# LeadRDRK/ZPack

Hardware: AMD Instinct MI355X
Metric: decompressed GiB/s over all entries; % HBM roofline (higher is better)
Workload: dtype u8; 1 GPU; c2_lz4_64k; entries_per_gpu=100000, entries_total=100000, archive_image_bytes_this_rank=3543588472, archive_image_bytes_all_ranks=3543588472, method=lz4, level=0, class_mix=70/20/5/5 text/records/random/runs, parallelism=one batch per rank, no data-path collective, rehearsal_one_card=False, frames_by=liblz4/libzstd of the image, reference writer call sequence

## Files before the change

### zpack_amd/__init__.py

```python
import ctypes as C
import os

import numpy as np

HERE = os.path.dirname(os.path.abspath(__file__))
CODEC_SO = os.environ.get("ZPACK_AMD_CODEC_SO") or os.path.join(HERE, "libzpk_codec.so")
ZPACK_SO = os.path.join(HERE, "libzpack_amd.so")

METHOD_NONE, METHOD_ZSTD, METHOD_LZ4 = 0, 1, 2
DF_SKIP_HASH = 1
DF_GENERAL = 2
K_CLASSIFY, K_STORED, K_LZ4, K_ZSTD, K_ZSTD_FSE, K_PACK, K_ENCODE = 0, 1, 2, 3, 4, 5, 7
OPT_ENC_SPLIT_MIN, OPT_DEC_SPLIT_MIN, OPT_ORDER_MIN, OPT_ORDER_FAST_LAST = 6, 7, 8, 9

DECODE_DESC = np.dtype([("src_offset", "<u8"), ("comp_size", "<u8"), ("uncomp_size", "<u8"), ("expect_hash", "<u8"),
                        ("dst_offset", "<u8"), ("dst_capacity", "<u8"), ("method", "<u4"), ("flags", "<u4")])
DECODE_RESULT = np.dtype([("status", "<i4"), ("detail", "<u4"), ("produced", "<u8"), ("hash", "<u8")])
ENCODE_DESC = np.dtype([("src_offset", "<u8"), ("size", "<u8"), ("dst_offset", "<u8"), ("dst_capacity", "<u8"),
                        ("method", "<u4"), ("level", "<i4")])
ENCODE_RESULT = np.dtype([("status", "<i4"), ("detail", "<u4"), ("comp_size", "<u8"), ("hash", "<u8")])
assert DECODE_DESC.itemsize == 56 and DECODE_RESULT.itemsize == 24
assert ENCODE_DESC.itemsize == 40 and ENCODE_RESULT.itemsize == 24

_lib = None
# ... 121 lines not shown
        self._chk(self.L.zpk_codec_set_profiling(self.h, 1 if on else 0), "set_profiling")

    def kernel_ms(self, which):
        ms = C.c_float(0)
        self._chk(self.L.zpk_codec_kernel_ms(self.h, which, C.byref(ms)), "kernel_ms")
        return ms.value

    def decode_stats(self):
        a = (C.c_uint32 * 8)()
        self._chk(self.L.zpk_codec_decode_stats(self.h, a), "decode_stats")
        b = (C.c_uint32 * 16)()
        self.L.zpk_codec_decode_stats2.argtypes = [C.c_void_p, C.POINTER(C.c_uint32)]
        self._chk(self.L.zpk_codec_decode_stats2(self.h, b), "decode_stats2")
        return dict(stored=a[0], zstd=a[1], lz4=a[2], zstd_two_stage=a[3], zstd_fused=a[4], fse_watchdog=a[5], fse_budget=a[6],
                    zstd_arena_refused=bool(a[7] >> 31), retried_lz4=b[0], retried_zstd=b[1],
                    lz4_long_runs=b[3],
                    frame_parallel_entries=b[5], frame_parallel_frames=b[6], zstd_blocks_flags=b[7])

    def debug_fetch(self, what, offset, count, dtype):
        a = np.zeros(count, dtype=dtype)
        self._chk(self.L.zpk_codec_debug_fetch(self.h, what, offset, a.ctypes.data, a.nbytes), "debug_fetch")
        return a

    def debug_read(self, n):
        a = np.zeros((n, 8), dtype=np.uint64)
        self._chk(self.L.zpk_codec_debug_read(self.h, a.ctypes.data, a.nbytes), "debug_read")
        return a

    def timer_start(self, stream=None):
        self._chk(self.L.zpk_codec_timer_start(self.h, C.c_void_p(stream) if stream else None), "timer_start")

# ... 44 lines not shown
```

### zpack_amd/csrc/lz4_wave.h

```cpp
#pragma once
#include "zpk_device.h"
#include "xxh3_device.h"
#include "seq_exec.h"

namespace zpk {

__device__ __noinline__ u32 window_word(const u8* a, const u8* lo, const u8* hi)
{
    if (a >= lo && a + 4 <= hi) return ld32(a);
    u32 v = 0;
    #pragma unroll
    for (int i = 0; i < 4; i++) if (a + i >= lo && a + i < hi) v |= (u32)ld8(a + i) << (8 * i);
    return v;
}

struct ByteWindow {
    u32 w;
    const u8* base;
    const u8* lo;
    const u8* hi;

    __device__ __forceinline__ void load(const u8* p, int lane)
    {
        base = (const u8*)((u64)p & ~(u64)3);
// ... 380 lines not shown
        if (cck) {
            if (iend - ip < 4) { r.rc = D_TRUNCATED; r.produced = (u64)(op - dst); return r; }
            u32 h = 0;
            lane0_guard();
            if (lane == 0) h = xxh32_serial(frame_out, (u64)(op - frame_out), 0);
            if (uni(h) != uld32(ip)) { r.rc = D_MALFORMED; return r; }
            ip += 4;
        }
        if (has_cs && content_size != (u64)(op - frame_out)) { r.rc = D_MALFORMED; return r; }
        if (rs) { rs->nframes++; rs->in_blocks = 0; rs->frame_ip_off = (u64)(ip - src); rs->frame_op_off = (u64)(op - dst); }
    }
    r.produced = (u64)(op - dst);
    return r;
}

}
```

### zpack_amd/csrc/zpk_codec.hip

```cpp
#include <hip/hip_runtime.h>
#include <stdio.h>
#include <stdlib.h>
#include <string.h>
#include <new>
#include <time.h>
#include <pthread.h>
#include <thread>
#include <atomic>
#include <vector>
#include <algorithm>


#include "zpk_device.h"
#include "xxh3_device.h"
#include "xxh3_span.h"
#include "lz4_wave.h"
#include "lx_ring.h"
#ifndef LX_WAVES_PER_SIMD
#define LX_WAVES_PER_SIMD 6
#endif
#include "zstd_wg.h"
#include "zstd_fse4.h"
#include "zstd_ring.h"
#include "lz4_pj.h"
#include "zstd_pj.h"
#include "host_walk.h"

using namespace zpk;

enum { L_NONE = 0, L_ZSTD = 1, L_LZ4 = 2, L_COUNT = 4, N_LISTS = 3, L_LZ4_RUNS = 100  };
enum { C_ZSTD_TWO_STAGE = 9, C_ZSTD_FUSED = 10, C_EXEC_HEAD = 16, C_LEFT_COUNT = 17,
       C_RETRY_LZ4 = 18, C_RETRY_ZSTD = 19,
       C_RETRY_HEAD = 20,
       C_LZ4_LEFT = 21, C_LZ4_LEFT_HEAD = 22,
       C_ENC_CLASS = 28,
       C_ORDER_SPAN = 26,
       C_ORDER = 32,
       N_COUNTERS = 32 + 64 };
enum { N_LISTS_ALLOC = N_LISTS + 5 };


#define ORD_CLASSES 16
__device__ __forceinline__ int order_class(u64 size)
{
    const int lg = 63 - __clzll((long long)(size | 1));
    const int b = 26 - lg;
    return b < 0 ? 0 : (b > ORD_CLASSES - 1 ? ORD_CLASSES - 1 : b);
}
__device__ __forceinline__ int order_fast(u64 size, u64 comp) { return comp * 16 >= size * 15 ? 1 : 0; }
__global__ __launch_bounds__(256) void k_classify(const zpk_decode_desc* __restrict__ desc, u64 n, u64 src_size, u64 dst_size,
                                                  zpk_decode_result* __restrict__ res, u32* __restrict__ lists, u64 list_stride,
                                                  u32* __restrict__ counters)
{
    u64 i = (u64)blockIdx.x * blockDim.x + threadIdx.x;
    const bool live = i < n;
    zpk_decode_desc d; memset(&d, 0, sizeof(d));
    if (live) d = desc[i];
    zpk_decode_result r; r.status = R_OK; r.detail = 0; r.produced = 0; r.hash = 0;
    int list = -1;
    if (!live) list = -1;
    else if (d.comp_size == 0) r.status = R_OK;
    else if (d.dst_capacity < d.uncomp_size) r.status = R_BUFFER_TOO_SMALL;
    else if (d.src_offset + d.comp_size >= src_size || d.src_offset > src_size || d.comp_size > src_size - d.src_offset)
        r.status = R_FILE_OFFSET_INVALID;
    else if (d.dst_offset > dst_size || d.dst_capacity > dst_size - d.dst_offset) { r.status = R_BUFFER_TOO_SMALL; r.detail = 0xBAD0D57u; }
    else if (d.method == ZPK_METHOD_NONE) {
        if (d.uncomp_size > d.comp_size) r.status = R_FILE_SIZE_INVALID;
        else list = L_NONE;
    }
    else if (d.method == ZPK_METHOD_ZSTD) list = L_ZSTD;
    else if (d.method == ZPK_METHOD_LZ4) list = d.comp_size < (d.uncomp_size >> 3) ? L_LZ4_RUNS : L_LZ4;
    else r.status = R_COMP_METHOD_INVALID;
    if (list >= 0) { r.status = R_DECOMPRESS_FAILED; r.detail = 0xFFFFFFFFu; }
    if (live) res[i] = r;
    const int lane = lane_id();
    {
        const bool dec = list == L_ZSTD || list == L_LZ4;
        u32 hi = dec ? (u32)order_class(d.uncomp_size) + 1u : 0u, inv = dec ? (u32)(ORD_CLASSES - order_class(d.uncomp_size)) : 0u;
        #pragma unroll
        for (int m = 1; m < 64; m <<= 1) { const u32 a = (u32)__shfl_xor((int)hi, m, 64), b2 = (u32)__shfl_xor((int)inv, m, 64); hi = a > hi ? a : hi; inv = b2 > inv ? b2 : inv; }
        if (lane == 0 && hi) { atomicMax(&counters[C_ORDER_SPAN], hi - 1u); atomicMax(&counters[C_ORDER_SPAN + 1], inv - 1u); }
    }
    #pragma unroll
    for (int L = 0; L < N_LISTS; L++) {
        const u64 m = __ballot(list == L);
        if (m == 0) continue;
        const int leader = __ffsll((long long)m) - 1;
        u32 base = 0;
        if (lane == leader) base = atomicAdd(&counters[L], (u32)__popcll(m));
        base = (u32)__shfl((int)base, leader, 64);
        if (list == L) lists[(u64)L * list_stride + base + (u32)__popcll(m & ((1ull << lane) - 1))] = (u32)i;
    }
    {
        const u64 m = __ballot(list == L_LZ4_RUNS);
        if (m != 0) {
            const int leader = __ffsll((long long)m) - 1;
            u32 base = 0;
            if (lane == leader) base = atomicAdd(&counters[C_LZ4_LEFT], (u32)__popcll(m));
            base = (u32)__shfl((int)base, leader, 64);
            if (list == L_LZ4_RUNS) lists[(u64)(N_LISTS + 2) * list_stride + base + (u32)__popcll(m & ((1ull << lane) - 1))] = (u32)i;
        }
    }
}

__device__ __forceinline__ bool order_single_class(const u32* counters) { return counters[C_ORDER_SPAN] + counters[C_ORDER_SPAN + 1] == ORD_CLASSES - 1; }
__device__ __forceinline__ void order_wave_rank(int b, int lane, u32& rank, u32& count)
{
    rank = 0; count = 0;
    u64 todo = __ballot(b >= 0);
    while (todo) {
        const int cls = __shfl(b, __ffsll((long long)todo) - 1, 64);
        const u64 m = __ballot(b == cls);
        if (b == cls) { rank = (u32)__popcll(m & ((1ull << lane) - 1)); count = (u32)__popcll(m); }
        todo &= ~m;
    }
}
__global__ __launch_bounds__(256) void k_order_count(const zpk_decode_desc* __restrict__ desc, const u32* __restrict__ lists, u64 list_stride,
                                                     u32* __restrict__ counters, int fast_last)
{
    __shared__ u32 h[ORD_CLASSES];
    const int L = blockIdx.y == 0 ? L_ZSTD : L_LZ4;
    const u32 cnt = counters[L];
    const bool uniform = order_single_class(counters);
    if ((u64)blockIdx.x * 256 >= cnt || (uniform && !fast_last)) return;
    if (threadIdx.x < ORD_CLASSES) h[threadIdx.x] = 0;
    __syncthreads();
    const u64 k = (u64)blockIdx.x * 256 + threadIdx.x;
    const int lane = lane_id();
    int b = -1;
    if (k < cnt) { const zpk_decode_desc& d = desc[lists[(u64)L * list_stride + k]]; b = uniform ? order_fast(d.uncomp_size, d.comp_size) : order_class(d.uncomp_size); }
    u32 rank, count;
    order_wave_rank(b, lane, rank, count);
    if (b >= 0 && rank == 0) atomicAdd(&h[b], count);
    __syncthreads();
    if (threadIdx.x < ORD_CLASSES && h[threadIdx.x]) atomicAdd(&counters[C_ORDER + blockIdx.y * ORD_CLASSES + threadIdx.x], h[threadIdx.x]);
}
__global__ __launch_bounds__(256) void k_order_fill(const zpk_decode_desc* __restrict__ desc, const u32* __restrict__ lists, u64 list_stride,
                                                    u32* __restrict__ ordered , u32* __restrict__ counters, int fast_last)
{
    __shared__ u32 wcount[4][ORD_CLASSES], base[ORD_CLASSES];
    const int L = blockIdx.y == 0 ? L_ZSTD : L_LZ4;
    const u32 cnt = counters[L];
    if ((u64)blockIdx.x * 256 >= cnt) return;
    const u64 k = (u64)blockIdx.x * 256 + threadIdx.x;
    const bool uniform = order_single_class(counters);
    if (uniform && !fast_last) { if (k < cnt) ordered[(u64)blockIdx.y * list_stride + k] = lists[(u64)L * list_stride + k]; return; }
    if (threadIdx.x < 4 * ORD_CLASSES) (&wcount[0][0])[threadIdx.x] = 0;
    __syncthreads();
    const int lane = lane_id(), w = threadIdx.x >> 6;
    u32 e = 0; int b = -1;
    if (k < cnt) { e = lists[(u64)L * list_stride + k]; b = uniform ? order_fast(desc[e].uncomp_size, desc[e].comp_size) : order_class(desc[e].uncomp_size); }
    u32 rank, count;
    order_wave_rank(b, lane, rank, count);
    if (b >= 0 && rank == 0) wcount[w][b] = count;
    __syncthreads();
    if (threadIdx.x < ORD_CLASSES) {
        const int c = threadIdx.x;
        const u32 total = wcount[0][c] + wcount[1][c] + wcount[2][c] + wcount[3][c];
        const u32* const hist = counters + C_ORDER + blockIdx.y * ORD_CLASSES;
        u32 before = 0;
        for (int j = 0; j < c; j++) before += hist[j];
        base[c] = total ? before + atomicAdd(&counters[C_ORDER + 2 * ORD_CLASSES + blockIdx.y * ORD_CLASSES + c], total) : 0;
    }
    __syncthreads();
    if (b >= 0) {
        u32 at = base[b] + rank;
        for (int j = 0; j < w; j++) at += wcount[j][b];
        ordered[(u64)blockIdx.y * list_stride + at] = e;
    }
}

__device__ __forceinline__ bool my_slot(const u32* counters, int list, u32& idx)
{
    idx = uni((u32)(((u64)blockIdx.x * blockDim.x + threadIdx.x) >> 6));
    return idx < uni(counters[list]);
}

__device__ __forceinline__ void finish_entry(const zpk_decode_desc& d, zpk_decode_result* res, u32 e, int status, u32 detail,
                                             u64 produced, const u8* out, int lane)
{
    u64 h = 0;
    lane0_guard();
    if (status == R_OK) {
// ... 46 lines not shown
            const u64 done = nblocks << 10;
            for (u64 i = done + lane; i < len; i += WAVE) st8(out + i, ld8(in + i));
            const u32 nstripes = (u32)(((len - 1) - done) >> 6);
            h = st.finish(in + done, nstripes, in + len, len, lane);
        }
        int status = R_OK;
        if (!(d.flags & ZPK_DF_SKIP_HASH) && h != d.expect_hash) status = R_FILE_HASH_MISMATCH;
        lane0_guard();
        if (lane == 0) {
            zpk_decode_result r; r.status = status; r.detail = 0; r.produced = len; r.hash = h;
            res[e] = r;
        }
    }
}

template <int COOP>
__device__ __forceinline__ void lz4_entry_wave(Lz4WaveShared& shw, const u8* __restrict__ src, const u8* read_lo, const u8* read_hi,
                                               const zpk_decode_desc* __restrict__ desc, u8* dst, zpk_decode_result* __restrict__ res,
                                               u32 e, u32* __restrict__ counters, u64* __restrict__ dbg, u32* __restrict__ retry_list,
                                               u32 wd_scale, int lane)
{
    const zpk_decode_desc d = desc[e];
    const u8* in = uni_ptr(src + d.src_offset);
    u8* out = uni_ptr(dst + d.dst_offset);
    Watchdog wd; wd.arm(uni64(d.comp_size) + uni64(d.dst_capacity), wd_scale);
    SeqStats stt = {};
    const u64 t_all = SEQ_T(); (void)t_all;
    DecodeOut o = lz4f_decode_wave<COOP>(shw, wd, stt, in, uni64(d.comp_size), read_lo, read_hi, out, uni64(d.dst_capacity), lane);
#ifdef ZPK_STATS
    if (dbg && lane == 0) {
        u64* g = dbg + (u64)e * 8;
        g[0] = stt.t_parse; g[1] = stt.t_lit; g[2] = stt.t_dep; g[3] = stt.t_rounds;
        g[4] = ((u64)stt.batches << 32) | stt.rounds; g[5] = ((u64)stt.coops << 32) | stt.asm_batches; g[6] = SEQ_T() - t_all;
        g[7] = ((u64)stt.fix_iters << 32) | stt.chunks;
#ifdef ZPK_STATS_PARSE
        g[0] = stt.t_stage; g[1] = stt.t_walk1; g[2] = stt.t_fix; g[3] = stt.t_emit; g[4] = stt.t_tok;
        g[5] = ((u64)stt.hops_first << 32) | stt.hops_fix; g[6] = stt.slow_hops;
#endif
    }
#else
    (void)dbg; (void)t_all;
#endif
    if (wd.fired && retry_list) {
        lane0_guard();
        if (lane == 0) retry_list[atomicAdd(&counters[C_RETRY_LZ4], 1u)] = e;
        return;
    }
    int status = R_OK;
    if (o.rc == D_MALFORMED) status = R_DECOMPRESS_FAILED;
    else if (o.rc == D_TRUNCATED) status = o.produced < d.dst_capacity ? R_FILE_INCOMPLETE : R_BUFFER_TOO_SMALL;
    else if (o.rc == D_DST_FULL) status = R_BUFFER_TOO_SMALL;
    finish_entry(d, res, e, status, wd.fired ? 0xDEADu : (u32)(-o.rc), o.produced, out, lane);
}

__global__ __launch_bounds__(64, 8) void k_lz4_wave(const u8* __restrict__ src, const u8* read_lo, const u8* read_hi,
                                                  const zpk_decode_desc* __restrict__ desc, u8* dst,
                                                  zpk_decode_result* __restrict__ res, const u32* __restrict__ list,
                                                  u32* __restrict__ counters, u64* __restrict__ dbg, u32* __restrict__ retry_list
#ifdef ZPK_DEVELOPER
                                                  , u32 wd_scale
#endif
                                                  )
{
#ifndef ZPK_DEVELOPER
    const u32 wd_scale = 1u;
#endif
    const int lane = lane_id();
    __shared__ Lz4WaveShared shw;
    u32 idx;
    if (my_slot(counters, L_LZ4, idx))
        lz4_entry_wave<0>(shw, src, read_lo, read_hi, desc, dst, res, uni(list[idx]), counters, dbg, retry_list, wd_scale, lane);
}

__global__ __launch_bounds__(64, 8) void k_lz4_retry(const u8* __restrict__ src, const u8* read_lo, const u8* read_hi,
                                                   const zpk_decode_desc* __restrict__ desc, u8* dst,
                                                   zpk_decode_result* __restrict__ res, const u32* __restrict__ list,
                                                   u32* __restrict__ counters, u64* __restrict__ dbg)
{
    const int lane = lane_id();
    __shared__ Lz4WaveShared shw;
    const u32 n_slots = uni(counters[C_RETRY_LZ4]);
    for (u32 idx = uni((u32)blockIdx.x); idx < n_slots; idx += gridDim.x)
        lz4_entry_wave<2>(shw, src, read_lo, read_hi, desc, dst, res, uni(list[idx]), counters, dbg, nullptr, (u32)ZPK_WATCHDOG_RETRY_SCALE, lane);
}

#define LZ4_LEFT_GRID_MAX 8192u
#ifndef LZ4_LEFT_WAVES
#define LZ4_LEFT_WAVES 8
#endif
__global__ __launch_bounds__(64, LZ4_LEFT_WAVES) void k_lz4_left(const u8* __restrict__ src, const u8* read_lo, const u8* read_hi,
                                                  const zpk_decode_desc* __restrict__ desc, u8* dst,
                                                  zpk_decode_result* __restrict__ res, const u32* __restrict__ list,
                                                  u32* __restrict__ counters, u64* __restrict__ dbg, u32* __restrict__ retry_list, u32 wd_scale)
{
    const int lane = lane_id();
    __shared__ Lz4WaveShared shw;
    const u32 n_slots = uni(counters[C_LZ4_LEFT]);
    if (n_slots == 0) return;
// ... 341 lines not shown
    CodecLock lk(c);
    (void)hipSetDevice(c->device);
    (void)hipStreamSynchronize(c->stream);
    (void)hipGetLastError();
    c->err[0] = 0;
    const u64 keep = 64ull << 20;
    void** bufs[] = { (void**)&c->d_src, (void**)&c->d_dst, (void**)&c->d_zarena, (void**)&c->d_lit };
    u64* caps[] = { &c->src_cap, &c->dst_cap, &c->zarena_cap, &c->lit_cap };
    for (int i = 0; i < 5; i++) if (*bufs[i] && *caps[i] > keep) { (void)hipFree(*bufs[i]); *bufs[i] = nullptr; *caps[i] = 0; }
}
const char* zpk_codec_last_error(const zpk_codec* c) { return c ? c->err : "no codec"; }
int zpk_codec_device(const zpk_codec* c) { return c ? c->device : -1; }

#ifdef ZPK_DEVELOPER
#define ZPK_DEV(x) x
#define ZPK_WD_ARG , wd_scale
#else
#define ZPK_DEV(x)
#define ZPK_WD_ARG
#endif

static int xxh3_spans_launch(zpk_codec* c, const u8* base, const zpk_span* h_spans, u64 nspans, u64 part_blocks, u64* h_hash, hipStream_t st)
{
    if (nspans == 0) return ZPK_OK;
    if (nspans > 0x7FFFFFFFull) return ZPK_E_INVALID;
    const u64 span_bytes = (nspans * sizeof(zpk_span) + 255) & ~255ull, part_bytes = part_blocks * 64;
    int rc;
    if ((rc = grow(c, (void**)&c->d_xpart, &c->xpart_cap, span_bytes + part_bytes + nspans * 8 + 64))) return rc;
    zpk_span* d_spans = (zpk_span*)c->d_xpart;
    u64* d_part = (u64*)(c->d_xpart + span_bytes);
    u64* d_hash = (u64*)(c->d_xpart + span_bytes + part_bytes);
// ... 7 lines not shown
}
static inline u64 xxh3_span_blocks(u64 len) { return (((len - 1) >> 10) + XS_GROUP - 1) / XS_GROUP * XS_GROUP; }

static int decode_launch(zpk_codec* c, const u8* src, u64 src_size, const u8* read_lo, const u8* read_hi,
                         const zpk_decode_desc* desc, u64 n, u8* dst, u64 dst_size, zpk_decode_result* res, hipStream_t st)
{
    if (n == 0) return ZPK_OK;
    if (n > 0x7FFFFFF0ull) return ZPK_E_INVALID;
    c->totals_valid = 0;
    int rc;
    if ((rc = grow(c, (void**)&c->d_lists, &c->list_cap, N_LISTS_ALLOC * n * sizeof(u32)))) return rc;
    const u64 stride = c->list_cap / (N_LISTS_ALLOC * sizeof(u32));
    u32* const retry_lz4 = c->d_lists + (u64)N_LISTS * stride;
    u32* const retry_zstd = c->d_lists + (u64)(N_LISTS + 1) * stride;
    u32* const left_lz4 = c->d_lists + (u64)(N_LISTS + 2) * stride;
    u32 wd_scale = 1; (void)wd_scale;
    ZPK_DEV(static const int wd_env = getenv("ZPK_WD_SCALE") ? atoi(getenv("ZPK_WD_SCALE")) : 1; wd_scale = (u32)wd_env;)
    int skip = 0; (void)skip;
#ifdef ZPK_DEVELOPER
    static const int want_dbg = getenv("ZPK_DEBUG_TIMING") ? atoi(getenv("ZPK_DEBUG_TIMING")) : 0;
    if (want_dbg) { if ((rc = grow(c, (void**)&c->d_dbg, &c->dbg_cap, n * 128))) return rc; }
    static const int trace = getenv("ZPK_TRACE") ? atoi(getenv("ZPK_TRACE")) : 0;
    static const int skip_env = getenv("ZPK_SKIP") ? atoi(getenv("ZPK_SKIP")) : 0;
    skip = skip_env;
#define ZPK_TRACE_STEP(name) do { if (trace == 1) { hipError_t te_ = hipStreamSynchronize(st); \
        fprintf(stderr, "[zpk] %s done: %s\n", name, hipGetErrorString(te_)); fflush(stderr); } } while (0)
#else
#define ZPK_TRACE_STEP(name) do { } while (0)
#endif
    const u32 zstd_grid = (u32)(n < ZSTD_GRID_MAX ? n : ZSTD_GRID_MAX);
    const u32 exec_grid = (u32)(n < ZSTD_EXEC_GRID_MAX ? n : ZSTD_EXEC_GRID_MAX);
    const bool maybe_zstd = c->zstd_hint != 0;
    if (maybe_zstd && (rc = grow(c, (void**)&c->d_lit, &c->lit_cap, (u64)(exec_grid > zstd_grid ? exec_grid : zstd_grid) * ZSTD_LIT_SCRATCH))) return rc;
    HIPCHK(c, hipMemsetAsync(c->d_counters, 0, N_COUNTERS * sizeof(u32), st));
    ZPK_TRACE_STEP("memset");
#define ZPK_KEV(k, j) do { if (c->profiling) (void)hipEventRecord(c->kev[k][j], st); } while (0)
    ZPK_KEV(ZPK_K_CLASSIFY, 0);
    hipLaunchKernelGGL(k_classify, dim3((u32)((n + 255) / 256)), dim3(256), 0, st, desc, n, src_size, dst_size, res,
                       c->d_lists, stride, c->d_counters);
    const u32* zstd_list = c->d_lists + L_ZSTD * stride;
    const u32* lz4_list = c->d_lists + L_LZ4 * stride;
    if (n >= c->order_min) {
        u32* const ordered = c->d_lists + (u64)(N_LISTS + 3) * stride;
        const dim3 og((u32)((n + 255) / 256), 2);
        hipLaunchKernelGGL(k_order_count, og, dim3(256), 0, st, desc, (const u32*)c->d_lists, stride, c->d_counters, c->order_fast_last);
        hipLaunchKernelGGL(k_order_fill, og, dim3(256), 0, st, desc, (const u32*)c->d_lists, stride, ordered, c->d_counters, c->order_fast_last);
        zstd_list = ordered; lz4_list = ordered + stride;
    }
    ZPK_KEV(ZPK_K_CLASSIFY, 1);
    ZPK_TRACE_STEP("k_classify");
    const u32 wgrid = (u32)((n + 3) / 4);
    ZPK_KEV(ZPK_K_STORED, 0);
    if (!(skip & 1)) hipLaunchKernelGGL(k_stored, dim3(wgrid), dim3(256), 0, st, src, desc, dst, res, c->d_lists + L_NONE * stride, c->d_counters);
    ZPK_KEV(ZPK_K_STORED, 1);
    ZPK_TRACE_STEP("k_stored");
    const bool maybe_lz4 = c->lz4_hint != 0;
    hipStream_t sl = st;
#ifndef ZPK_NO_SIDE_STREAM
    if (!c->h_seen && hipHostMalloc((void**)&c->h_seen, 64, hipHostMallocDefault) == hipSuccess) { c->h_seen[L_NONE] = 0; c->h_seen[L_ZSTD] = 1; c->h_seen[L_LZ4] = 1; c->h_seen[8] = 1; }
    const bool both_seen = c->zstd_hint >= 0  || (c->h_seen && c->h_seen[L_ZSTD] != 0 && c->h_seen[L_LZ4] != 0);
    if (maybe_lz4 && maybe_zstd && both_seen && !(skip & 6)) {
        int lo_prio = 0, hi_prio = 0;
        if (!c->s_side) { (void)hipDeviceGetStreamPriorityRange(&lo_prio, &hi_prio);
                          if (hipStreamCreateWithPriority(&c->s_side, hipStreamNonBlocking, lo_prio) != hipSuccess) c->s_side = nullptr; }
        if (!c->ev_fork && hipEventCreateWithFlags(&c->ev_fork, hipEventDisableTiming) != hipSuccess) c->ev_fork = nullptr;
        if (!c->ev_join && hipEventCreateWithFlags(&c->ev_join, hipEventDisableTiming) != hipSuccess) c->ev_join = nullptr;
        if (c->s_side && c->ev_fork && c->ev_join && hipEventRecord(c->ev_fork, st) == hipSuccess &&
            hipStreamWaitEvent(c->s_side, c->ev_fork, 0) == hipSuccess) sl = c->s_side;
    }
#endif
    auto launch_lz4 = [&]() {
        if (c->profiling) (void)hipEventRecord(c->kev[ZPK_K_LZ4][0], sl);
        if (!(skip & 2) && maybe_lz4) {
            hipStream_t sx = sl;
            if (n >= 4096 && c->h_seen && c->h_seen[8] != 0) {
            if (!c->s_left && hipStreamCreateWithFlags(&c->s_left, hipStreamNonBlocking) != hipSuccess) c->s_left = nullptr;
            if (!c->ev_lfork && hipEventCreateWithFlags(&c->ev_lfork, hipEventDisableTiming) != hipSuccess) c->ev_lfork = nullptr;
            if (!c->ev_ljoin && hipEventCreateWithFlags(&c->ev_ljoin, hipEventDisableTiming) != hipSuccess) c->ev_ljoin = nullptr;
            if (c->s_left && c->ev_lfork && c->ev_ljoin && hipEventRecord(c->ev_lfork, sl) == hipSuccess &&
                hipStreamWaitEvent(c->s_left, c->ev_lfork, 0) == hipSuccess) sx = c->s_left;
            }
            hipLaunchKernelGGL(k_lz4_left, dim3((u32)(n < LZ4_LEFT_GRID_MAX ? n : LZ4_LEFT_GRID_MAX)), dim3(64), 0, sx, src, read_lo, read_hi, desc, dst, res,
                               (const u32*)left_lz4, c->d_counters, c->d_dbg, retry_lz4, wd_scale);
            hipLaunchKernelGGL(k_lz4_wave, dim3((u32)n), dim3(64), 0, sl, src, read_lo, read_hi, desc, dst, res,
                               lz4_list, c->d_counters, c->d_dbg, retry_lz4 ZPK_WD_ARG);
            if (sx != sl && (hipEventRecord(c->ev_ljoin, sx) != hipSuccess || hipStreamWaitEvent(sl, c->ev_ljoin, 0) != hipSuccess))
                (void)hipStreamSynchronize(sx);
            hipLaunchKernelGGL(k_lz4_retry, dim3((u32)(n < 256 ? n : 256)), dim3(64), 0, sl, src, read_lo, read_hi, desc, dst, res,
                               (const u32*)retry_lz4, c->d_counters, c->d_dbg);
        }
        if (c->profiling) (void)hipEventRecord(c->kev[ZPK_K_LZ4][1], sl);
    };
    if (sl == st) launch_lz4();
    ZPK_TRACE_STEP("k_lz4_wave");
    bool two_stage = maybe_zstd && dst_size >= 64;
    ZPK_DEV(static const int fused_only = getenv("ZPK_ZSTD_FUSED") ? atoi(getenv("ZPK_ZSTD_FUSED")) : 0; if (fused_only) two_stage = false;)
    c->fell_back_fused = 0;
    if (two_stage && (grow(c, (void**)&c->d_zarena, &c->zarena_cap, dst_size + 64) != ZPK_OK ||
                      grow(c, (void**)&c->d_zstate, &c->zstate_cap, 2 * n * sizeof(u32)) != ZPK_OK)) {
        two_stage = false; c->fell_back_fused = 1;
        snprintf(c->err, sizeof(c->err), "note: no memory for the %llu-byte Zstandard sequence arena; this batch ran the fused decoder",
                 (unsigned long long)dst_size + 64);
    }
    u32* const leftover = two_stage ? c->d_zstate + n : nullptr;
// ... 15 lines not shown
                       two_stage ? (const u32*)leftover : zstd_list, c->d_counters, c->d_lit, c->d_dbg,
                       two_stage ? (int)C_LEFT_COUNT : (int)L_ZSTD, (int)(L_COUNT + L_ZSTD), retry_zstd, (int)C_RETRY_ZSTD, wd_scale);
    ZPK_KEV(ZPK_K_ZSTD, 1);
    ZPK_TRACE_STEP("k_zstd");
    if (!(skip & 4) && maybe_zstd)
        hipLaunchKernelGGL(k_zstd, dim3(zstd_grid < 128 ? zstd_grid : 128), dim3(ZSTD_WG_THREADS), 0, st, src, desc, dst, res,
                           (const u32*)retry_zstd, c->d_counters, c->d_lit, c->d_dbg, (int)C_RETRY_ZSTD, (int)C_RETRY_HEAD,
                           (u32*)nullptr, 0, (u32)ZPK_WATCHDOG_RETRY_SCALE);
    if (sl != st) {
        launch_lz4();
        if (hipEventRecord(c->ev_join, sl) != hipSuccess || hipStreamWaitEvent(st, c->ev_join, 0) != hipSuccess) {
            (void)hipStreamSynchronize(sl);
        }
    }
    ZPK_TRACE_STEP("retry");
    if (c->h_seen && c->zstd_hint < 0) (void)hipMemcpyAsync((void*)c->h_seen, c->d_counters, N_LISTS * sizeof(u32), hipMemcpyDeviceToHost, st);
    if (c->h_seen) (void)hipMemcpyAsync((void*)(c->h_seen + 8), c->d_counters + C_LZ4_LEFT, sizeof(u32), hipMemcpyDeviceToHost, st);
    HIPCHK(c, hipGetLastError());
    return ZPK_OK;
}

int zpk_codec_decode_batch_device(zpk_codec* c, const uint8_t* src, uint64_t src_size, const zpk_decode_desc* desc, uint64_t n,
                                  uint8_t* dst, uint64_t dst_size, zpk_decode_result* results, void* stream)
{
    if (!c || (n && (!desc || !results))) return ZPK_E_INVALID;
    CodecLock lk(c);
    HIPCHK(c, hipSetDevice(c->device));
    hipStream_t st = stream ? (hipStream_t)stream : c->stream;
    c->zstd_hint = -1; c->lz4_hint = -1;
    return decode_launch(c, src, src_size, src, src + src_size, desc, n, dst, dst_size, results, st);
}
// ... 869 lines not shown
{
    if (!c || !c->d_dbg || bytes > c->dbg_cap) return ZPK_E_INVALID;
    HIPCHK(c, hipDeviceSynchronize());
    HIPCHK(c, hipMemcpy(host, c->d_dbg, bytes, hipMemcpyDeviceToHost));
    return ZPK_OK;
}

int zpk_codec_decode_stats(zpk_codec* c, uint32_t out[8])
{
    if (!c || !out) return ZPK_E_INVALID;
    HIPCHK(c, hipSetDevice(c->device));
    HIPCHK(c, hipDeviceSynchronize());
    u32 h[N_COUNTERS];
    HIPCHK(c, hipMemcpy(h, c->d_counters, sizeof(h), hipMemcpyDeviceToHost));
    if (c->totals_valid) memcpy(h, c->host_totals, sizeof(h));
    out[0] = h[L_NONE]; out[1] = h[L_ZSTD]; out[2] = h[L_LZ4] + h[C_LZ4_LEFT] ; out[3] = h[C_ZSTD_TWO_STAGE]; out[4] = h[C_ZSTD_FUSED];
    out[5] = h[ZF_WATCHDOG_WORD]; out[6] = h[ZF_WATCHDOG_WORD + 1]; out[7] = h[13];
    if (c->fell_back_fused) out[7] |= 0x80000000u;
    ZPK_DEV(if (getenv("ZPK_TRACE")) fprintf(stderr, "[zpk] fse marked %u, pass-0 failures %u, last failure status/rc %08x\n", h[13], h[14], h[15]);)
    return ZPK_OK;
}

int zpk_codec_decode_stats2(zpk_codec* c, uint32_t out[16])
{
    if (!c || !out) return ZPK_E_INVALID;
    CodecLock lk(c);
    HIPCHK(c, hipSetDevice(c->device));
    HIPCHK(c, hipDeviceSynchronize());
    u32 h[N_COUNTERS];
    HIPCHK(c, hipMemcpy(h, c->d_counters, sizeof(h), hipMemcpyDeviceToHost));
    if (c->totals_valid) memcpy(h, c->host_totals, sizeof(h));
    memset(out, 0, 16 * sizeof(uint32_t));
    out[0] = h[C_RETRY_LZ4]; out[1] = h[C_RETRY_ZSTD];
    out[2] = 0; out[3] = h[C_LZ4_LEFT]; out[4] = 0;
    out[5] = c->big_last[0]; out[6] = c->big_last[1];
    out[7] = c->zpj_last_err;
    return ZPK_OK;
}

int zpk_codec_debug_fetch(zpk_codec* c, int what, uint64_t offset, void* host, uint64_t bytes)
{
    if (!c || !host) return ZPK_E_INVALID;
    const u8* base = what == 0 ? (const u8*)c->d_zarena : (const u8*)c->d_zstate;
    const u64 cap = what == 0 ? c->zarena_cap : c->zstate_cap;
    if (!base || offset > cap || bytes > cap - offset) return ZPK_E_INVALID;
    HIPCHK(c, hipSetDevice(c->device));
    HIPCHK(c, hipDeviceSynchronize());
    HIPCHK(c, hipMemcpy(host, base + offset, bytes, hipMemcpyDeviceToHost));
    return ZPK_OK;
}

// ... 52 lines not shown
```

Measured before the change: 624.6 GiB/s.

## Split LZ4 decode into lean plain-frame path and general fallback kernel

Classification now inspects each LZ4 frame header and sends common plain frames (no checksums, no dict, default flags) to a slimmed k_lz4_wave that uses a specialized lz4f_plain_wave decoder. Other frames go to a new k_lz4_general persistent kernel. Entries the lean path rejects are handed to the retry kernel, which now drains three queues. The goal is less per-entry branching and register pressure on the common path, at the cost of an extra kernel launch, more list slots and counters, and a reading of source headers during classification.

```diff
diff --git a/zpack_amd/__init__.py b/zpack_amd/__init__.py
--- a/zpack_amd/__init__.py
+++ b/zpack_amd/__init__.py
@@ -159,7 +159,7 @@
         self._chk(self.L.zpk_codec_decode_stats2(self.h, b), "decode_stats2")
         return dict(stored=a[0], zstd=a[1], lz4=a[2], zstd_two_stage=a[3], zstd_fused=a[4], fse_watchdog=a[5], fse_budget=a[6],
                     zstd_arena_refused=bool(a[7] >> 31), retried_lz4=b[0], retried_zstd=b[1],
-                    lz4_long_runs=b[3],
+                    lz4_long_runs=b[3], lz4_handed_over=b[8], lz4_general=b[9],
                     frame_parallel_entries=b[5], frame_parallel_frames=b[6], zstd_blocks_flags=b[7])
 
     def debug_fetch(self, what, offset, count, dtype):
diff --git a/zpack_amd/csrc/lz4_wave.h b/zpack_amd/csrc/lz4_wave.h
--- a/zpack_amd/csrc/lz4_wave.h
+++ b/zpack_amd/csrc/lz4_wave.h
@@ -418,4 +418,51 @@
     return r;
 }
 
-}
+template <int COOP = 0>
+__device__ inline bool lz4f_plain_wave(Lz4WaveShared& sh, Watchdog& wd, SeqStats& stt, const u8* src, u64 src_size, const u8* src_hi,
+                                       u8* dst, u64 dst_cap, u64 want, int lane)
+{
+    if (src_size < 11) return false;
+    if (uld32(src) != 0x184D2204u) return false;
+    const u32 flg = uld8(src + 4), bd = uld8(src + 5);
+    if ((flg & 0xD7u) != 0x40u || (bd & 0x8Fu) || ((bd >> 4) & 7u) < 4u) return false;
+    const u32 hdr = (flg & 8u) ? 15u : 7u;
+    if (src_size < hdr + 4u) return false;
+    if ((flg & 8u) && uni64(ld64(src + 6)) != want) return false;
+    {
+        u32 h = 0;
+        lane0_guard();
+        if (lane == 0) h = (xxh32_serial(src + 4, hdr - 5, 0) >> 8) & 0xFF;
+        if (uni(h) != uld8(src + hdr - 1)) return false;
+    }
+    const u64 bmax = (u64)1 << (8 + 2 * ((bd >> 4) & 7u));
+    const bool indep = (flg >> 5) & 1;
+    const u8* ip = src + hdr;
+    const u8* const iend = src + src_size;
+    u8* op = dst;
+    u8* const oend = dst + dst_cap;
+    for (;;) {
+        if (wd.expired() || iend - ip < 4) return false;
+        const u32 bh = uld32(ip);
+        ip += 4;
+        if (bh == 0) break;
+        const u32 bsz = bh & 0x7FFFFFFFu;
+        if (bsz > bmax || (u64)(iend - ip) < bsz) return false;
+        if (bh >> 31) {
+            if (bsz > (u64)(oend - op)) return false;
+            for (u32 i = (u32)lane * 16; i < bsz; i += WAVE * 16) gcopy_upto16(op + i, ip + i, bsz - i < 16 ? bsz - i : 16);
+            op += bsz;
+        } else {
+            u8* hist_lo = indep ? op : dst;
+            if ((u64)(op - hist_lo) > 65536) hist_lo = op - 65536;
+            u8* bend = oend;
+            if ((u64)(oend - op) > bmax) bend = op + bmax;
+            if (lz4_block_wave<COOP>(sh, wd, stt, ip, bsz, src_hi, hist_lo, op, bend, lane) != D_OK) return false;
+        }
+        wave_mem_fence();
+        ip += bsz;
+    }
+    return ip == iend && (u64)(op - dst) == want;
+}
+
+}
diff --git a/zpack_amd/csrc/zpk_codec.hip b/zpack_amd/csrc/zpk_codec.hip
--- a/zpack_amd/csrc/zpk_codec.hip
+++ b/zpack_amd/csrc/zpk_codec.hip
@@ -28,16 +28,24 @@
 
 using namespace zpk;
 
-enum { L_NONE = 0, L_ZSTD = 1, L_LZ4 = 2, L_COUNT = 4, N_LISTS = 3, L_LZ4_RUNS = 100  };
+enum { L_NONE = 0, L_ZSTD = 1, L_LZ4 = 2, L_COUNT = 4, N_LISTS = 3, L_LZ4_RUNS = 100 ,
+       L_LZ4_GEN = 101  };
 enum { C_ZSTD_TWO_STAGE = 9, C_ZSTD_FUSED = 10, C_EXEC_HEAD = 16, C_LEFT_COUNT = 17,
        C_RETRY_LZ4 = 18, C_RETRY_ZSTD = 19,
        C_RETRY_HEAD = 20,
        C_LZ4_LEFT = 21, C_LZ4_LEFT_HEAD = 22,
+       C_LZ4_GEN = 3, C_LZ4_GEN_HEAD = 7,
+       C_LZ4_HANDED_HEAD = 23, C_LZ4_HANDED = 24,
+       C_LZ4_RETRY_HEAD = 25,
        C_ENC_CLASS = 28,
        C_ORDER_SPAN = 26,
        C_ORDER = 32,
-       N_COUNTERS = 32 + 64 };
-enum { N_LISTS_ALLOC = N_LISTS + 5 };
+       N_COUNTERS = 32 + 96 };
+enum { S_LZ4_HANDED = N_LISTS + 5, S_LZ4_GEN = N_LISTS + 6, S_LZ4_GEN_ORDERED = N_LISTS + 7, N_LISTS_ALLOC = N_LISTS + 8 };
+#define N_ORDERED 3
+__device__ __forceinline__ int order_list_slot(int y) { return y == 0 ? (int)L_ZSTD : y == 1 ? (int)L_LZ4 : (int)S_LZ4_GEN; }
+__device__ __forceinline__ int order_count_word(int y) { return y == 0 ? (int)L_ZSTD : y == 1 ? (int)L_LZ4 : (int)C_LZ4_GEN; }
+__device__ __forceinline__ int order_out_slot(int y) { return y == 2 ? (int)S_LZ4_GEN_ORDERED : (int)N_LISTS + 3 + y; }
 
 
 #define ORD_CLASSES 16
@@ -48,7 +56,13 @@
     return b < 0 ? 0 : (b > ORD_CLASSES - 1 ? ORD_CLASSES - 1 : b);
 }
 __device__ __forceinline__ int order_fast(u64 size, u64 comp) { return comp * 16 >= size * 15 ? 1 : 0; }
-__global__ __launch_bounds__(256) void k_classify(const zpk_decode_desc* __restrict__ desc, u64 n, u64 src_size, u64 dst_size,
+__device__ __forceinline__ bool lz4_header_is_plain(const u8* __restrict__ p, u64 comp_size)
+{
+    if (comp_size < 11) return false;
+    const u32 magic = (u32)p[0] | ((u32)p[1] << 8) | ((u32)p[2] << 16) | ((u32)p[3] << 24), flg = p[4], bd = p[5];
+    return magic == 0x184D2204u && (flg & 0xD7u) == 0x40u && (bd & 0x8Fu) == 0 && ((bd >> 4) & 7u) >= 4u;
+}
+__global__ __launch_bounds__(256) void k_classify(const u8* __restrict__ src, const zpk_decode_desc* __restrict__ desc, u64 n, u64 src_size, u64 dst_size,
                                                   zpk_decode_result* __restrict__ res, u32* __restrict__ lists, u64 list_stride,
                                                   u32* __restrict__ counters)
 {
@@ -69,13 +83,14 @@
         else list = L_NONE;
     }
     else if (d.method == ZPK_METHOD_ZSTD) list = L_ZSTD;
-    else if (d.method == ZPK_METHOD_LZ4) list = d.comp_size < (d.uncomp_size >> 3) ? L_LZ4_RUNS : L_LZ4;
+    else if (d.method == ZPK_METHOD_LZ4)
+        list = d.comp_size < (d.uncomp_size >> 3) ? L_LZ4_RUNS : lz4_header_is_plain(src + d.src_offset, d.comp_size) ? L_LZ4 : L_LZ4_GEN;
     else r.status = R_COMP_METHOD_INVALID;
     if (list >= 0) { r.status = R_DECOMPRESS_FAILED; r.detail = 0xFFFFFFFFu; }
     if (live) res[i] = r;
     const int lane = lane_id();
     {
-        const bool dec = list == L_ZSTD || list == L_LZ4;
+        const bool dec = list == L_ZSTD || list == L_LZ4 || list == L_LZ4_GEN;
         u32 hi = dec ? (u32)order_class(d.uncomp_size) + 1u : 0u, inv = dec ? (u32)(ORD_CLASSES - order_class(d.uncomp_size)) : 0u;
         #pragma unroll
         for (int m = 1; m < 64; m <<= 1) { const u32 a = (u32)__shfl_xor((int)hi, m, 64), b2 = (u32)__shfl_xor((int)inv, m, 64); hi = a > hi ? a : hi; inv = b2 > inv ? b2 : inv; }
@@ -101,6 +116,16 @@
             if (list == L_LZ4_RUNS) lists[(u64)(N_LISTS + 2) * list_stride + base + (u32)__popcll(m & ((1ull << lane) - 1))] = (u32)i;
         }
     }
+    {
+        const u64 m = __ballot(list == L_LZ4_GEN);
+        if (m != 0) {
+            const int leader = __ffsll((long long)m) - 1;
+            u32 base = 0;
+            if (lane == leader) base = atomicAdd(&counters[C_LZ4_GEN], (u32)__popcll(m));
+            base = (u32)__shfl((int)base, leader, 64);
+            if (list == L_LZ4_GEN) lists[(u64)S_LZ4_GEN * list_stride + base + (u32)__popcll(m & ((1ull << lane) - 1))] = (u32)i;
+        }
+    }
 }
 
 __device__ __forceinline__ bool order_single_class(const u32* counters) { return counters[C_ORDER_SPAN] + counters[C_ORDER_SPAN + 1] == ORD_CLASSES - 1; }
@@ -119,8 +144,8 @@
                                                      u32* __restrict__ counters, int fast_last)
 {
     __shared__ u32 h[ORD_CLASSES];
-    const int L = blockIdx.y == 0 ? L_ZSTD : L_LZ4;
-    const u32 cnt = counters[L];
+    const int L = order_list_slot(blockIdx.y);
+    const u32 cnt = counters[order_count_word(blockIdx.y)];
     const bool uniform = order_single_class(counters);
     if ((u64)blockIdx.x * 256 >= cnt || (uniform && !fast_last)) return;
     if (threadIdx.x < ORD_CLASSES) h[threadIdx.x] = 0;
@@ -136,15 +161,16 @@
     if (threadIdx.x < ORD_CLASSES && h[threadIdx.x]) atomicAdd(&counters[C_ORDER + blockIdx.y * ORD_CLASSES + threadIdx.x], h[threadIdx.x]);
 }
 __global__ __launch_bounds__(256) void k_order_fill(const zpk_decode_desc* __restrict__ desc, const u32* __restrict__ lists, u64 list_stride,
-                                                    u32* __restrict__ ordered , u32* __restrict__ counters, int fast_last)
+                                                    u32* __restrict__ all_lists , u32* __restrict__ counters, int fast_last)
 {
     __shared__ u32 wcount[4][ORD_CLASSES], base[ORD_CLASSES];
-    const int L = blockIdx.y == 0 ? L_ZSTD : L_LZ4;
-    const u32 cnt = counters[L];
+    const int L = order_list_slot(blockIdx.y);
+    const u32 cnt = counters[order_count_word(blockIdx.y)];
+    u32* const ordered = all_lists + (u64)order_out_slot(blockIdx.y) * list_stride;
     if ((u64)blockIdx.x * 256 >= cnt) return;
     const u64 k = (u64)blockIdx.x * 256 + threadIdx.x;
     const bool uniform = order_single_class(counters);
-    if (uniform && !fast_last) { if (k < cnt) ordered[(u64)blockIdx.y * list_stride + k] = lists[(u64)L * list_stride + k]; return; }
+    if (uniform && !fast_last) { if (k < cnt) ordered[k] = lists[(u64)L * list_stride + k]; return; }
     if (threadIdx.x < 4 * ORD_CLASSES) (&wcount[0][0])[threadIdx.x] = 0;
     __syncthreads();
     const int lane = lane_id(), w = threadIdx.x >> 6;
@@ -160,13 +186,13 @@
         const u32* const hist = counters + C_ORDER + blockIdx.y * ORD_CLASSES;
         u32 before = 0;
         for (int j = 0; j < c; j++) before += hist[j];
-        base[c] = total ? before + atomicAdd(&counters[C_ORDER + 2 * ORD_CLASSES + blockIdx.y * ORD_CLASSES + c], total) : 0;
+        base[c] = total ? before + atomicAdd(&counters[C_ORDER + N_ORDERED * ORD_CLASSES + blockIdx.y * ORD_CLASSES + c], total) : 0;
     }
     __syncthreads();
     if (b >= 0) {
         u32 at = base[b] + rank;
         for (int j = 0; j < w; j++) at += wcount[j][b];
-        ordered[(u64)blockIdx.y * list_stride + at] = e;
+        ordered[at] = e;
     }
 }
 
@@ -243,19 +269,8 @@
     }
 }
 
-template <int COOP>
-__device__ __forceinline__ void lz4_entry_wave(Lz4WaveShared& shw, const u8* __restrict__ src, const u8* read_lo, const u8* read_hi,
-                                               const zpk_decode_desc* __restrict__ desc, u8* dst, zpk_decode_result* __restrict__ res,
-                                               u32 e, u32* __restrict__ counters, u64* __restrict__ dbg, u32* __restrict__ retry_list,
-                                               u32 wd_scale, int lane)
-{
-    const zpk_decode_desc d = desc[e];
-    const u8* in = uni_ptr(src + d.src_offset);
-    u8* out = uni_ptr(dst + d.dst_offset);
-    Watchdog wd; wd.arm(uni64(d.comp_size) + uni64(d.dst_capacity), wd_scale);
-    SeqStats stt = {};
-    const u64 t_all = SEQ_T(); (void)t_all;
-    DecodeOut o = lz4f_decode_wave<COOP>(shw, wd, stt, in, uni64(d.comp_size), read_lo, read_hi, out, uni64(d.dst_capacity), lane);
+__device__ __forceinline__ void lz4_stats_out(u64* __restrict__ dbg, u32 e, const SeqStats& stt, u64 t_all, int lane)
+{
 #ifdef ZPK_STATS
     if (dbg && lane == 0) {
         u64* g = dbg + (u64)e * 8;
@@ -268,8 +283,24 @@
 #endif
     }
 #else
-    (void)dbg; (void)t_all;
-#endif
+    (void)dbg; (void)e; (void)stt; (void)t_all; (void)lane;
+#endif
+}
+
+template <int COOP>
+__device__ __forceinline__ void lz4_entry_wave(Lz4WaveShared& shw, const u8* __restrict__ src, const u8* read_lo, const u8* read_hi,
+                                               const zpk_decode_desc* __restrict__ desc, u8* dst, zpk_decode_result* __restrict__ res,
+                                               u32 e, u32* __restrict__ counters, u64* __restrict__ dbg, u32* __restrict__ retry_list,
+                                               u32 wd_scale, int lane)
+{
+    const zpk_decode_desc d = desc[e];
+    const u8* in = uni_ptr(src + d.src_offset);
+    u8* out = uni_ptr(dst + d.dst_offset);
+    Watchdog wd; wd.arm(uni64(d.comp_size) + uni64(d.dst_capacity), wd_scale);
+    SeqStats stt = {};
+    const u64 t_all = SEQ_T(); (void)t_all;
+    DecodeOut o = lz4f_decode_wave<COOP>(shw, wd, stt, in, uni64(d.comp_size), read_lo, read_hi, out, uni64(d.dst_capacity), lane);
+    lz4_stats_out(dbg, e, stt, t_all, lane);
     if (wd.fired && retry_list) {
         lane0_guard();
         if (lane == 0) retry_list[atomicAdd(&counters[C_RETRY_LZ4], 1u)] = e;
@@ -282,35 +313,102 @@
     finish_entry(d, res, e, status, wd.fired ? 0xDEADu : (u32)(-o.rc), o.produced, out, lane);
 }
 
-__global__ __launch_bounds__(64, 8) void k_lz4_wave(const u8* __restrict__ src, const u8* read_lo, const u8* read_hi,
+__device__ __forceinline__ void lz4_entry_plain(Lz4WaveShared& shw, const u8* __restrict__ src, const u8* read_hi,
+                                                const zpk_decode_desc* __restrict__ desc, u8* dst, zpk_decode_result* __restrict__ res,
+                                                u32 e, u32* __restrict__ counters, u64* __restrict__ dbg, u32* __restrict__ retry_list,
+                                                u32* __restrict__ handed_list, u32 wd_scale, int lane)
+{
+    const zpk_decode_desc& d = desc[e];
+    const u8* in = uni_ptr(src + d.src_offset);
+    u8* out = uni_ptr(dst + d.dst_offset);
+    Watchdog wd; wd.arm(uni64(d.comp_size) + uni64(d.dst_capacity), wd_scale);
+    SeqStats stt = {};
+    const u64 t_all = SEQ_T(); (void)t_all;
+    const bool done = lz4f_plain_wave<0>(shw, wd, stt, in, uni64(d.comp_size), read_hi, out, uni64(d.dst_capacity), uni64(d.uncomp_size), lane);
+    lz4_stats_out(dbg, e, stt, t_all, lane);
+    if (!done) {
+        lane0_guard();
+        if (lane == 0) {
+            if (wd.fired) retry_list[atomicAdd(&counters[C_RETRY_LZ4], 1u)] = e;
+            else handed_list[atomicAdd(&counters[C_LZ4_HANDED], 1u)] = e;
+        }
+        return;
+    }
+    finish_entry(d, res, e, R_OK, 0u, uni64(d.uncomp_size), out, lane);
+}
+
+__global__ __launch_bounds__(64, 8) void k_lz4_wave(const u8* __restrict__ src, const u8* read_hi,
                                                   const zpk_decode_desc* __restrict__ desc, u8* dst,
                                                   zpk_decode_result* __restrict__ res, const u32* __restrict__ list,
-                                                  u32* __restrict__ counters, u64* __restrict__ dbg, u32* __restrict__ retry_list
+                                                  u32* __restrict__ counters, u32* __restrict__ retry_list, u32* __restrict__ handed_list
 #ifdef ZPK_DEVELOPER
-                                                  , u32 wd_scale
+                                                  , u64* __restrict__ dbg, u32 wd_scale
 #endif
                                                   )
 {
 #ifndef ZPK_DEVELOPER
     const u32 wd_scale = 1u;
+    u64* const dbg = nullptr;
 #endif
     const int lane = lane_id();
     __shared__ Lz4WaveShared shw;
     u32 idx;
     if (my_slot(counters, L_LZ4, idx))
+        lz4_entry_plain(shw, src, read_hi, desc, dst, res, uni(list[idx]), counters, dbg, retry_list, handed_list, wd_scale, lane);
+}
+
+#ifdef ZPK_DEVELOPER
+__global__ __launch_bounds__(256) void k_lz4_hand_all(const u32* __restrict__ list, u32* __restrict__ counters, u32* __restrict__ handed_list)
+{
+    const u64 i = (u64)blockIdx.x * blockDim.x + threadIdx.x;
+    if (i < counters[L_LZ4]) handed_list[atomicAdd(&counters[C_LZ4_HANDED], 1u)] = list[i];
+}
+#endif
+
+#define LZ4_GENERAL_GRID_MAX 8192u
+__global__ __launch_bounds__(64, 8) void k_lz4_general(const u8* __restrict__ src, const u8* read_lo, const u8* read_hi,
+                                                     const zpk_decode_desc* __restrict__ desc, u8* dst,
+                                                     zpk_decode_result* __restrict__ res, const u32* __restrict__ list,
+                                                     u32* __restrict__ counters, u64* __restrict__ dbg, u32* __restrict__ retry_list, u32 wd_scale)
+{
+    const int lane = lane_id();
+    __shared__ Lz4WaveShared shw;
+    const u32 n_slots = uni(counters[C_LZ4_GEN]);
+    if (n_slots == 0) return;
+    for (;;) {
+        lane0_guard();
+        u32 v = 0;
+        if (lane == 0) v = atomicAdd(&counters[C_LZ4_GEN_HEAD], 1u);
+        const u32 idx = uni(v);
+        lane0_guard();
+        if (idx >= n_slots) break;
         lz4_entry_wave<0>(shw, src, read_lo, read_hi, desc, dst, res, uni(list[idx]), counters, dbg, retry_list, wd_scale, lane);
+    }
 }
 
 __global__ __launch_bounds__(64, 8) void k_lz4_retry(const u8* __restrict__ src, const u8* read_lo, const u8* read_hi,
                                                    const zpk_decode_desc* __restrict__ desc, u8* dst,
-                                                   zpk_decode_result* __restrict__ res, const u32* __restrict__ list,
-                                                   u32* __restrict__ counters, u64* __restrict__ dbg)
+                                                   zpk_decode_result* __restrict__ res, const u32* __restrict__ lists, u64 list_stride,
+                                                   u32* __restrict__ counters, u64* __restrict__ dbg, int gen_slot)
 {
     const int lane = lane_id();
     __shared__ Lz4WaveShared shw;
-    const u32 n_slots = uni(counters[C_RETRY_LZ4]);
-    for (u32 idx = uni((u32)blockIdx.x); idx < n_slots; idx += gridDim.x)
-        lz4_entry_wave<2>(shw, src, read_lo, read_hi, desc, dst, res, uni(list[idx]), counters, dbg, nullptr, (u32)ZPK_WATCHDOG_RETRY_SCALE, lane);
+    for (int k = 0; k < 3; k++) {
+        const int count_word = k == 0 ? (int)C_LZ4_GEN : k == 1 ? (int)C_LZ4_HANDED : (int)C_RETRY_LZ4;
+        const int head_word = k == 0 ? (int)C_LZ4_GEN_HEAD : k == 1 ? (int)C_LZ4_HANDED_HEAD : (int)C_LZ4_RETRY_HEAD;
+        const u32* const list = lists + (u64)(k == 0 ? gen_slot : k == 1 ? (int)S_LZ4_HANDED : (int)N_LISTS) * list_stride;
+        const u32 n_slots = uni(counters[count_word]);
+        if (n_slots == 0 || uni(counters[head_word]) >= n_slots) continue;
+        for (;;) {
+            lane0_guard();
+            u32 v = 0;
+            if (lane == 0) v = atomicAdd(&counters[head_word], 1u);
+            const u32 idx = uni(v);
+            lane0_guard();
+            if (idx >= n_slots) break;
+            lz4_entry_wave<2>(shw, src, read_lo, read_hi, desc, dst, res, uni(list[idx]), counters, dbg, nullptr, (u32)ZPK_WATCHDOG_RETRY_SCALE, lane);
+        }
+    }
 }
 
 #define LZ4_LEFT_GRID_MAX 8192u
@@ -682,7 +780,7 @@
 
 #ifdef ZPK_DEVELOPER
 #define ZPK_DEV(x) x
-#define ZPK_WD_ARG , wd_scale
+#define ZPK_WD_ARG , c->d_dbg, wd_scale
 #else
 #define ZPK_DEV(x)
 #define ZPK_WD_ARG
@@ -720,6 +818,7 @@
     u32* const retry_lz4 = c->d_lists + (u64)N_LISTS * stride;
     u32* const retry_zstd = c->d_lists + (u64)(N_LISTS + 1) * stride;
     u32* const left_lz4 = c->d_lists + (u64)(N_LISTS + 2) * stride;
+    u32* const handed_lz4 = c->d_lists + (u64)S_LZ4_HANDED * stride;
     u32 wd_scale = 1; (void)wd_scale;
     ZPK_DEV(static const int wd_env = getenv("ZPK_WD_SCALE") ? atoi(getenv("ZPK_WD_SCALE")) : 1; wd_scale = (u32)wd_env;)
     int skip = 0; (void)skip;
@@ -742,17 +841,19 @@
     ZPK_TRACE_STEP("memset");
 #define ZPK_KEV(k, j) do { if (c->profiling) (void)hipEventRecord(c->kev[k][j], st); } while (0)
     ZPK_KEV(ZPK_K_CLASSIFY, 0);
-    hipLaunchKernelGGL(k_classify, dim3((u32)((n + 255) / 256)), dim3(256), 0, st, desc, n, src_size, dst_size, res,
+    hipLaunchKernelGGL(k_classify, dim3((u32)((n + 255) / 256)), dim3(256), 0, st, src, desc, n, src_size, dst_size, res,
                        c->d_lists, stride, c->d_counters);
     const u32* zstd_list = c->d_lists + L_ZSTD * stride;
     const u32* lz4_list = c->d_lists + L_LZ4 * stride;
+    int gen_slot = S_LZ4_GEN;
     if (n >= c->order_min) {
-        u32* const ordered = c->d_lists + (u64)(N_LISTS + 3) * stride;
-        const dim3 og((u32)((n + 255) / 256), 2);
+        const dim3 og((u32)((n + 255) / 256), N_ORDERED);
         hipLaunchKernelGGL(k_order_count, og, dim3(256), 0, st, desc, (const u32*)c->d_lists, stride, c->d_counters, c->order_fast_last);
-        hipLaunchKernelGGL(k_order_fill, og, dim3(256), 0, st, desc, (const u32*)c->d_lists, stride, ordered, c->d_counters, c->order_fast_last);
-        zstd_list = ordered; lz4_list = ordered + stride;
-    }
+        hipLaunchKernelGGL(k_order_fill, og, dim3(256), 0, st, desc, (const u32*)c->d_lists, stride, c->d_lists, c->d_counters, c->order_fast_last);
+        zstd_list = c->d_lists + (u64)(N_LISTS + 3) * stride; lz4_list = c->d_lists + (u64)(N_LISTS + 4) * stride;
+        gen_slot = S_LZ4_GEN_ORDERED;
+    }
+    const u32* const gen_list = c->d_lists + (u64)gen_slot * stride;
     ZPK_KEV(ZPK_K_CLASSIFY, 1);
     ZPK_TRACE_STEP("k_classify");
     const u32 wgrid = (u32)((n + 3) / 4);
@@ -763,8 +864,8 @@
     const bool maybe_lz4 = c->lz4_hint != 0;
     hipStream_t sl = st;
 #ifndef ZPK_NO_SIDE_STREAM
-    if (!c->h_seen && hipHostMalloc((void**)&c->h_seen, 64, hipHostMallocDefault) == hipSuccess) { c->h_seen[L_NONE] = 0; c->h_seen[L_ZSTD] = 1; c->h_seen[L_LZ4] = 1; c->h_seen[8] = 1; }
-    const bool both_seen = c->zstd_hint >= 0  || (c->h_seen && c->h_seen[L_ZSTD] != 0 && c->h_seen[L_LZ4] != 0);
+    if (!c->h_seen && hipHostMalloc((void**)&c->h_seen, 64, hipHostMallocDefault) == hipSuccess) { c->h_seen[L_NONE] = 0; c->h_seen[L_ZSTD] = 1; c->h_seen[L_LZ4] = 1; c->h_seen[8] = 1; c->h_seen[C_LZ4_GEN] = 1; }
+    const bool both_seen = c->zstd_hint >= 0  || (c->h_seen && c->h_seen[L_ZSTD] != 0 && (c->h_seen[L_LZ4] != 0 || c->h_seen[C_LZ4_GEN] != 0));
     if (maybe_lz4 && maybe_zstd && both_seen && !(skip & 6)) {
         int lo_prio = 0, hi_prio = 0;
         if (!c->s_side) { (void)hipDeviceGetStreamPriorityRange(&lo_prio, &hi_prio);
@@ -788,12 +889,21 @@
             }
             hipLaunchKernelGGL(k_lz4_left, dim3((u32)(n < LZ4_LEFT_GRID_MAX ? n : LZ4_LEFT_GRID_MAX)), dim3(64), 0, sx, src, read_lo, read_hi, desc, dst, res,
                                (const u32*)left_lz4, c->d_counters, c->d_dbg, retry_lz4, wd_scale);
-            hipLaunchKernelGGL(k_lz4_wave, dim3((u32)n), dim3(64), 0, sl, src, read_lo, read_hi, desc, dst, res,
-                               lz4_list, c->d_counters, c->d_dbg, retry_lz4 ZPK_WD_ARG);
+            bool lean = true;
+#ifdef ZPK_DEVELOPER
+            static const int all_general = getenv("ZPK_LZ4_GENERAL") ? atoi(getenv("ZPK_LZ4_GENERAL")) : 0;
+            lean = !all_general;
+            if (!lean) hipLaunchKernelGGL(k_lz4_hand_all, dim3((u32)((n + 255) / 256)), dim3(256), 0, sl, lz4_list, c->d_counters, handed_lz4);
+#endif
+            if (lean) hipLaunchKernelGGL(k_lz4_wave, dim3((u32)n), dim3(64), 0, sl, src, read_hi, desc, dst, res,
+                                         lz4_list, c->d_counters, retry_lz4, handed_lz4 ZPK_WD_ARG);
+            if (!c->h_seen || c->h_seen[C_LZ4_GEN] != 0)
+                hipLaunchKernelGGL(k_lz4_general, dim3((u32)(n < LZ4_GENERAL_GRID_MAX ? n : LZ4_GENERAL_GRID_MAX)), dim3(64), 0, sl, src, read_lo, read_hi,
+                                   desc, dst, res, gen_list, c->d_counters, c->d_dbg, retry_lz4, wd_scale);
             if (sx != sl && (hipEventRecord(c->ev_ljoin, sx) != hipSuccess || hipStreamWaitEvent(sl, c->ev_ljoin, 0) != hipSuccess))
                 (void)hipStreamSynchronize(sx);
             hipLaunchKernelGGL(k_lz4_retry, dim3((u32)(n < 256 ? n : 256)), dim3(64), 0, sl, src, read_lo, read_hi, desc, dst, res,
-                               (const u32*)retry_lz4, c->d_counters, c->d_dbg);
+                               (const u32*)c->d_lists, stride, c->d_counters, c->d_dbg, gen_slot);
         }
         if (c->profiling) (void)hipEventRecord(c->kev[ZPK_K_LZ4][1], sl);
     };
@@ -839,7 +949,7 @@
         }
     }
     ZPK_TRACE_STEP("retry");
-    if (c->h_seen && c->zstd_hint < 0) (void)hipMemcpyAsync((void*)c->h_seen, c->d_counters, N_LISTS * sizeof(u32), hipMemcpyDeviceToHost, st);
+    if (c->h_seen && c->zstd_hint < 0) (void)hipMemcpyAsync((void*)c->h_seen, c->d_counters, (N_LISTS + 1) * sizeof(u32), hipMemcpyDeviceToHost, st);
     if (c->h_seen) (void)hipMemcpyAsync((void*)(c->h_seen + 8), c->d_counters + C_LZ4_LEFT, sizeof(u32), hipMemcpyDeviceToHost, st);
     HIPCHK(c, hipGetLastError());
     return ZPK_OK;
@@ -1739,7 +1849,7 @@
     u32 h[N_COUNTERS];
     HIPCHK(c, hipMemcpy(h, c->d_counters, sizeof(h), hipMemcpyDeviceToHost));
     if (c->totals_valid) memcpy(h, c->host_totals, sizeof(h));
-    out[0] = h[L_NONE]; out[1] = h[L_ZSTD]; out[2] = h[L_LZ4] + h[C_LZ4_LEFT] ; out[3] = h[C_ZSTD_TWO_STAGE]; out[4] = h[C_ZSTD_FUSED];
+    out[0] = h[L_NONE]; out[1] = h[L_ZSTD]; out[2] = h[L_LZ4] + h[C_LZ4_LEFT] + h[C_LZ4_GEN] ; out[3] = h[C_ZSTD_TWO_STAGE]; out[4] = h[C_ZSTD_FUSED];
     out[5] = h[ZF_WATCHDOG_WORD]; out[6] = h[ZF_WATCHDOG_WORD + 1]; out[7] = h[13];
     if (c->fell_back_fused) out[7] |= 0x80000000u;
     ZPK_DEV(if (getenv("ZPK_TRACE")) fprintf(stderr, "[zpk] fse marked %u, pass-0 failures %u, last failure status/rc %08x\n", h[13], h[14], h[15]);)
@@ -1760,6 +1870,8 @@
     out[2] = 0; out[3] = h[C_LZ4_LEFT]; out[4] = 0;
     out[5] = c->big_last[0]; out[6] = c->big_last[1];
     out[7] = c->zpj_last_err;
+    out[8] = h[C_LZ4_HANDED];
+    out[9] = h[C_LZ4_GEN];
     return ZPK_OK;
 }
 
```

Result: faster. 639.7 GiB/s, median of 6 (+2.4%).
